# theEricMa/TriplaneTurbo

Measured on AMD Instinct MI355X. Metric: rendered rays/sec (fwd+bwd) at 256x256 rays x 128 samples, higher is better.
Workload: dtype f32 (fp32-grade: exact 3-piece fp16 operand split, 6 x v_mfma_f32_32x32x16_f16 per k-step, fp32 accumulation)

## Files before the change

### triplaneturbo_amd/csrc/tt_backward.hip

```cpp
#include "tt_backward_common.h"

struct BwdGeoParams {
    const float* packed;
    MlpPtrs w;
    const float* rays_o;
    const float* rays_d;
    const float* t_starts;
    const float* t_ends;
    tt_render_cfg cfg;
    TileGeom geom;
    long long n_items;
    int* queue;
    const float* ws;
    int n_copies;
    float* grad_packed;
    MlpGradPtrs grads;
    unsigned long long* phase_cycles;
};

#define GEO_SCRATCH_FLOATS (2 * 64 * XS)
#define GOFF_W1T LDS_GEO_FLOATS
#define GOFF_W2T (GOFF_W1T + IMG16_FLOATS(32, 64))
#define LDS_GEO16_FLOATS (GOFF_W2T + IMG16_FLOATS(64, 64))
#define GLO_W1 LDS_GEO16_FLOATS
#define GLO_W2 (GLO_W1 + LO16_FLOATS(64, 32))
#define GLO_W1T (GLO_W2 + LO16_FLOATS(64, 64))
#define GLO_W2T (GLO_W1T + LO16_FLOATS(32, 64))
#define LDS_GEO3_FLOATS (GLO_W2T + LO16_FLOATS(64, 64))
template <int PREC>
struct GeoWFloats {
    static constexpr int value = PREC == PREC_S3 ? LDS_GEO3_FLOATS : LDS_GEO16_FLOATS;
};

template <int PREC, bool WG16, bool STATS = false>
__global__ __launch_bounds__(256, 1) void k_decode_bwd_geo(BwdGeoParams p) {
    constexpr bool EXACT = PREC == PREC_F32;
    constexpr int NT = PrecNT<PREC>::value, WF = GeoWFloats<PREC>::value;
    __shared__ __attribute__((aligned(16))) float L[WF + 4 * (GEO_SCRATCH_FLOATS + SCATTER_TAG_INTS)];
    {
        MlpPtrs w = p.w;
        stage_weights<PREC, 64, 32>(L + OFF_W1, L + GLO_W1, w.w1);
        stage_weights<PREC, 64, 64>(L + OFF_W2, L + GLO_W2, w.w2);
        lds_load_matrix(L + OFF_W3, w.w3, 1, 64, 64);
        stage_weights_t<PREC, 64, 32>(L + GOFF_W1T, L + GLO_W1T, w.w1);
        stage_weights_t<PREC, 64, 64>(L + GOFF_W2T, L + GLO_W2T, w.w2);
    }
    const tt_render_cfg& cfg = p.cfg;
    float sA1 = 1.f, sU = 1.f, sA2 = 1.f, sV = 1.f;
    if (WG16) {
        const unsigned* bnd = reinterpret_cast<const unsigned*>(p.queue) + TT_SLOT_BOUNDS;
        const float Pm = __builtin_bit_cast(float, bnd[TT_BOUND_PLANES]), Sb = __builtin_bit_cast(float, bnd[TT_BOUND_UP0]),
                    Gb = __builtin_bit_cast(float, bnd[TT_BOUND_UP1]);
        unsigned* word = reinterpret_cast<unsigned*>(L + WF);
        const int t = threadIdx.x;
        float w1row = 0.f, a1col = 0.f, w3abs = 0.f;
        if (t < 64) {
            for (int c = 0; c < 32; ++c) w1row += __builtin_fabsf(p.w.w1[t * 32 + c]);
            for (int r = 0; r < 64; ++r) a1col += __builtin_fabsf(p.w.w2[r * 64 + t]) * __builtin_fabsf(p.w.w3[r]);
            w3abs = __builtin_fabsf(p.w.w3[t]);
        }
        const float W1max = block_max(w1row, word), A1max = block_max(a1col, word), A2max = block_max(w3abs, word);
        const float jsum = (0.5f * cfg.plane_w + 0.5f * cfg.plane_h) / cfg.radius;
        const float Fmax = 3.f * Pm, H1max = W1max * Fmax;
        const float Umax = Fmax * (Sb + 2.f * jsum * Gb), QBmax = Fmax * 2.f * jsum * Gb;
        const float Vmax = Sb * H1max + W1max * QBmax;
        sA1 = wg16_scale(A1max);
        sU = wg16_scale(Umax);
        sA2 = wg16_scale(A2max);
        sV = wg16_scale(Vmax);
    }
    const TileGeom& tg = p.geom;
    const int lane = threadIdx.x & 63, i = lane & 31, hi = lane >> 5, wave_in_blk = threadIdx.x >> 6;
    float* Xs = L + WF + wave_in_blk * (GEO_SCRATCH_FLOATS + SCATTER_TAG_INTS);
    float* Ys = Xs + 64 * XS;
    int* tags = reinterpret_cast<int*>(Ys + 64 * XS);
    scatter_init_tags(tags, lane);
    __syncthreads();
    const int S = cfg.n_samples;
    ItemQueue iq = item_queue(p.queue, tg.n_blocks, tg.n_chunks, tg.unit);
    const int H = cfg.plane_h, W = cfg.plane_w;
    const size_t HW = (size_t)H * W;
    const size_t plane_stride = 6 * HW * TT_C;
    const float ju = 0.5f * W / cfg.radius, jv = 0.5f * H / cfg.radius;
    float* const grad_out =
        p.grad_packed + (size_t)(blockIdx.x % (unsigned)p.n_copies) * cfg.n_prompts * plane_stride;
    const unsigned grad_bytes =
        TT_DBG(cfg.flags, TT_DBG_NO_ATOMICS) ? 0u : (unsigned)(cfg.n_prompts * plane_stride * sizeof(float));

    const TileStats st = STATS ? tile_stats(cfg.stats) : TileStats{nullptr};
    f32x16 accW1[2][1] = {{ZERO16}, {ZERO16}};
    f32x16 accW2[2][2] = {{ZERO16, ZERO16}, {ZERO16, ZERO16}};
    float accw3 = 0.f;
#ifdef TT_TUNING
    unsigned long long ph_acc[20] = {0, 0, 0, 0, 0, 0, 0, 0, 0, 0, 0, 0, 0, 0, 0, 0, 0, 0, 0, 0};
    unsigned long long ph_t = __builtin_amdgcn_s_memtime();
#endif

#pragma nounroll
    for (;;) {
        long long b;
        int ck;
        if (!item_pop(iq, tg.order, tg.n_chunks, b, ck)) break;
        if (b >= tg.n_blocks) continue;
        bool ray_ok;
        const long long ray = tile_ray(tg, b, i, ray_ok);
        const float ray_okf = tt_opaque(ray_ok ? 1.f : 0.f);
        const int ks = i % tg.sb;
        const int view = (int)(ray / cfg.rays_per_view);
        const size_t pofs = (size_t)(view / cfg.views_per_prompt) * plane_stride;
        const float ox = p.rays_o[ray * 3 + 0], oy = p.rays_o[ray * 3 + 1], oz = p.rays_o[ray * 3 + 2];
        const float dx = p.rays_d ? p.rays_d[ray * 3 + 0] : 0.f, dy = p.rays_d ? p.rays_d[ray * 3 + 1] : 0.f,
                    dz = p.rays_d ? p.rays_d[ray * 3 + 2] : 0.f;
        const int s_end = (ck + 1) * tg.chunk < S ? (ck + 1) * tg.chunk : S;
        struct StepIn {
            f32x4 up;
            float ts, te;
        };
        auto load_step = [&](int sb0) {
            StepIn r;
            const int si = sb0 + ks;
            const long long sidx = ray * S + (si < S ? si : S - 1);
            r.up = *reinterpret_cast<const f32x4*>(p.ws + sidx * 4);
            r.ts = p.rays_d ? p.t_starts[sidx] : 0.f;
            r.te = p.rays_d ? p.t_ends[sidx] : 0.f;
            return r;
        };
        StepIn in = load_step(ck * tg.chunk), in_next;
#pragma nounroll
        for (int sb0 = ck * tg.chunk; sb0 < s_end; sb0 += tg.sb, in = in_next) {
            in_next = load_step(sb0 + tg.sb);
            const int si = sb0 + ks;
            const bool rvalid = ray_ok && si < s_end;
            const float vf = ray_okf * (si < s_end ? 1.f : 0.f);
            const float sbar = in.up[0] * vf, gbx = in.up[1] * vf, gby = in.up[2] * vf, gbz = in.up[3] * vf;
            tile_stat(st, TT_STAT_VISITED);
            TT_PHASE(0);
            if (!__any(!((__builtin_fabsf(sbar) + __builtin_fabsf(gbx)) + (__builtin_fabsf(gby) + __builtin_fabsf(gbz)) <=
                         cfg.skip_eps_geo)))
                continue;
            float tm, px, py, pz;
            sample_position(ox, oy, oz, dx, dy, dz, in.ts, in.te, tm, px, py, pz);
            const float X = scale_coord(px, cfg.radius), Y = scale_coord(py, cfg.radius),
                        Z = scale_coord(pz, cfg.radius);
            float f[16], u[16];
            bool anyp[3];
            const bool any = __any(gather_geo_bwd_c(p.packed, (unsigned)(pofs / TT_C), H, W, X, Y, Z, rvalid, sbar, gbx,
                                                    gby, gbz, ju, jv, lane, Xs, f, u, anyp,
                                                    tile_stat_ptr(st, TT_STAT_INBOUNDS)));
            TT_PHASE(1);
            if (!any) continue;
            tile_stat(st, TT_STAT_EXECUTED);
            float h1[32], h2[32], a2[32], a1[32], q[16], u1, u2;
            mvx<PREC, 64, 32, true>(L + OFF_W1, L + GLO_W1, f, h1, i, hi, 1.f, &u1);
#pragma unroll
            for (int r = 0; r < 32; ++r) h1[r] = fmaxf(h1[r], 0.f);
            mvx<PREC, 64, 64, true>(L + OFF_W2, L + GLO_W2, h1, h2, i, hi, u1, &u2);
#pragma unroll
            for (int r = 0; r < 32; ++r) h2[r] = fmaxf(h2[r], 0.f);
#pragma unroll
            for (int g = 0; g < 8; ++g) {
                f32x4 w3 = *reinterpret_cast<const f32x4*>(L + OFF_W3 + 8 * g + 4 * hi);
#pragma unroll
                for (int e2 = 0; e2 < 4; ++e2) a2[4 * g + e2] = h2[4 * g + e2] > 0.f ? w3[e2] : 0.f;
            }
            Split16<64, PAIR_SEQ, NT> a2s, a1s;
            float ua1 = 1.f;
            if (WG16) {
                split16_vec<64, PAIR_SEQ, NT>(a2, sA2, a2s);
                mv16_pre<64, 64, true, NT>(L + GOFF_W2T, a2s, 1.f / sA2, a1, i, hi, &ua1, L + GLO_W2T);
            } else {
                mvtx_copy<PREC, 64, 64, 64>(L + GOFF_W2T, L + GLO_W2T, L + OFF_W2, a2, a1, i, hi);
            }
#pragma unroll
            for (int r = 0; r < 32; ++r) a1[r] = h1[r] > 0.f ? a1[r] : 0.f;
            if (WG16) {
                split16_vec<64, PAIR_SEQ, NT>(a1, sA1 * ua1, a1s);
                mv16_pre<32, 64, false, NT>(L + GOFF_W1T, a1s, 1.f / sA1, q, i, hi, nullptr, L + GLO_W1T);
            } else {
                mvtx_copy<PREC, 32, 64, 32>(L + GOFF_W1T, L + GLO_W1T, L + OFF_W1, a1, q, i, hi);
            }
            TT_PHASE(3);
            {
                float qb[16];
#pragma unroll
                for (int r = 0; r < 16; ++r) qb[r] = fmaf(-sbar, f[r], u[r]);
                const bool region = WG16 ? true : cfg.flags >= 0;
                const bool do_wgrad = region && !TT_DBG(cfg.flags, TT_DBG_NO_WGRAD);
                if (do_wgrad) {
                    if (WG16) {
                        stage_rows16_pre<64>(Xs, a1s, i, hi);
                        stage_rows16<32>(Ys, u, i, hi, sU);
                        wgrad16<64, 32>(accW1, Xs, Ys, i, hi);
                    } else {
                        stage_rows<64>(Xs, a1, i, hi);
                        stage_rows<32>(Ys, u, i, hi);
                        wgrad<64, 32>(accW1, Xs, Ys, i, hi);
                    }
                }
                TT_PHASE(7);
                float t1[32];
                mvx<PREC, 64, 32>(L + OFF_W1, L + GLO_W1, qb, t1, i, hi);
#pragma unroll
                for (int r = 0; r < 32; ++r) t1[r] = h1[r] > 0.f ? t1[r] : 0.f;
                float v[32];
#pragma unroll
                for (int r = 0; r < 32; ++r) v[r] = fmaf(sbar * u1, h1[r], t1[r]);
                TT_PHASE(4);
                if (do_wgrad) {
                    if (WG16) {
                        stage_rows16_pre<64>(Xs, a2s, i, hi);
                        stage_rows16<64>(Ys, v, i, hi, sV);
                        wgrad16<64, 64>(accW2, Xs, Ys, i, hi);
                    } else {
                        stage_rows<64>(Xs, a2, i, hi);
                        stage_rows<64>(Ys, v, i, hi);
                        wgrad<64, 64>(accW2, Xs, Ys, i, hi);
                    }
                }
                TT_PHASE(8);
                float t2[32];
                mvx<PREC, 64, 64>(L + OFF_W2, L + GLO_W2, t1, t2, i, hi);
#pragma unroll
                for (int r = 0; r < 32; ++r) t2[r] = fmaf(sbar * u2, h2[r], h2[r] > 0.f ? t2[r] : 0.f);
                stage_rows<64>(Xs, t2, i, hi);
                accw3 += rowsum32(Xs, lane);
                TT_PHASE(5);
                if (region && !TT_DBG(cfg.flags, TT_DBG_NO_SCATTER)) {
                    scatter_clear<EXACT>(Xs, lane);
                    float* Qs = Xs + SCATTER_M_FLOATS;
                    TT_PHASE(9);
                    const int tex0 = (int)(pofs / TT_C);
                    scatter_planes<EXACT>(grad_out, grad_bytes, Qs, Xs, tags, Qs + 32 * 33, i, hi,
                                          [&](int pl, PlaneRefs& refs) {
                        Corners c;
                        float coef[4];
                        geo_corner_coefs(pl, H, W, X, Y, Z, rvalid, sbar, gbx, gby, gbz, ju, jv, c, coef);
                        int aoff[4];
#pragma unroll
                        for (int q4 = 0; q4 < 4; ++q4) aoff[q4] = tex0 + (int)(pl * HW) + c.off[q4];
                        refs = plane_refs<!EXACT>(coef, aoff, c.hs, hi);
#pragma unroll
                        for (int r = 0; r < 16; ++r) Qs[i * 33 + LIDX(r, hi)] = q[r] * refs.qs;
                    }
#ifdef TT_TUNING
                    , ph_acc + 14
#endif
                    );
                    TT_PHASE(10);
                }
            }
        }
    }
#ifdef TT_TUNING
    TT_PHASE(11);
    if (p.phase_cycles && lane == 0)
        for (int k = 0; k < 20; ++k) atomicAdd(p.phase_cycles + 20 + k, ph_acc[k]);
#endif
    __syncthreads();
    int parity = 0;
    flush_wgrad_reduced<64, 32>(L, parity, accW1, p.grads.w1, wave_in_blk, lane, 1.f / sA1, 1.f / sU);
    flush_wgrad_reduced<64, 64>(L, parity, accW2, p.grads.w2, wave_in_blk, lane, 1.f / sA2, 1.f / sV);
    atomicAdd(p.grads.w3 + lane, accw3);
    tile_stats_flush(st);
}

#ifdef TT_TUNING
unsigned long long* g_phase_cycles = nullptr;
extern "C" int tt_tuning_phase_cycles(unsigned long long* out40) {
    if (!g_phase_cycles) {
        if (hipMalloc((void**)&g_phase_cycles, 40 * sizeof(unsigned long long)) != hipSuccess) return -4;
        if (hipMemset(g_phase_cycles, 0, 40 * sizeof(unsigned long long)) != hipSuccess) return -4;
    }
    if (hipDeviceSynchronize() != hipSuccess) return -4;
    if (out40 && hipMemcpy(out40, g_phase_cycles, 40 * sizeof(unsigned long long), hipMemcpyDeviceToHost) != hipSuccess)
        return -4;
    return hipMemset(g_phase_cycles, 0, 40 * sizeof(unsigned long long)) == hipSuccess ? 0 : -4;
}
#endif
static void launch_bwd_geo(const BwdGeoParams& p0, long long blocks, hipStream_t s) {
    BwdGeoParams p = p0;
#ifdef TT_TUNING
    p.phase_cycles = g_phase_cycles;
#else
    p.phase_cycles = nullptr;
#endif
    const int prec = tt_prec_of_r(p.cfg.flags);
#define LAUNCH_GEO(PREC_, WG_)                                                                                        \
    do {                                                                                                              \
        if (p.cfg.stats)                                                                                              \
            hipLaunchKernelGGL((k_decode_bwd_geo<PREC_, WG_, true>), dim3((unsigned)blocks), dim3(256), 0, s, p);     \
        else                                                                                                          \
            hipLaunchKernelGGL((k_decode_bwd_geo<PREC_, WG_>), dim3((unsigned)blocks), dim3(256), 0, s, p);           \
    } while (0)
    if (use_wg16(p.cfg)) {
        unsigned* bnd = reinterpret_cast<unsigned*>(p.queue) + TT_SLOT_BOUNDS;
        launch_planes_bound(p.packed, p.cfg, 0, bnd + TT_BOUND_PLANES, s);
        const long long n = p.cfg.n_rays * p.cfg.n_samples;
        hipLaunchKernelGGL(k_absmax4, dim3(absmax_blocks(n), 1), dim3(256), 0, s, reinterpret_cast<const f32x4*>(p.ws), n, n,
                           bnd + TT_BOUND_UP0, bnd + TT_BOUND_UP1);
        if (prec == PREC_S3)
            LAUNCH_GEO(PREC_S3, true);
        else
            LAUNCH_GEO(PREC_S2, true);
    } else {
        LAUNCH_GEO(PREC_F32, false);
    }
#undef LAUNCH_GEO
}
int tt_launch_march_bwd(const float* rays_d, const float* t_starts, const float* t_ends, const tt_render_cfg* cfg,
                        const float* sdf, const float* sdf_grad, const float* features, const float* trans,
                        const float* opacity, const float* depth, const float* g_opacity, const float* g_depth,
                        const float* g_rgb_fg, const float* g_z_variance, const float* g_normal_acc,
                        const float* g_weights, const float* g_sdf, const float* g_sdf_grad, float* g_inv_std_rays,
                        float* ws, hipStream_t stream);

extern "C" int tt_render_bwd_geo(const float* packed, const tt_mlp_weights* w, const float* rays_o,
                                 const float* rays_d, const float* t_starts, const float* t_ends,
                                 const tt_render_cfg* cfg, const float* opacity, const float* depth,
                                 const float* trans, const float* sdf, const float* sdf_grad, const float* features,
                                 const float* g_opacity, const float* g_depth, const float* g_rgb_fg,
                                 const float* g_z_variance, const float* g_normal_acc, const float* g_weights,
                                 const float* g_sdf, const float* g_sdf_grad, float* g_inv_std_rays, float* workspace,
                                 float* grad_packed, const tt_mlp_grads* grads, void* stream) {
    int st = tt_validate_cfg(cfg);
    if (st != TT_OK) return st;
    if (!packed || !w || !rays_o || !rays_d || !t_starts || !t_ends || !opacity || !depth || !trans || !sdf ||
        !sdf_grad || !features || !workspace || !grad_packed || !grads)
        return TT_ERR_BAD_ARG;
    if (!w->w1 || !w->w2 || !w->w3 || !grads->w1 || !grads->w2 || !grads->w3) return TT_ERR_BAD_ARG;
    if (grad_buffer_too_large(cfg)) return TT_ERR_UNSUPPORTED;
    int cus = tt_num_cus();
    if (cus <= 0) return TT_ERR_DEVICE;
    hipStream_t s = (hipStream_t)stream;
    st = tt_launch_march_bwd(rays_d, t_starts, t_ends, cfg, sdf, sdf_grad, features, trans, opacity, depth, g_opacity,
                             g_depth, g_rgb_fg, g_z_variance, g_normal_acc, g_weights, g_sdf, g_sdf_grad, g_inv_std_rays,
                             workspace, s);
    if (st != TT_OK) return st;
    BwdGeoParams p;
    p.packed = packed;
    p.w = to_ptrs(w);
    p.rays_o = rays_o;
    p.rays_d = rays_d;
    p.t_starts = t_starts;
    p.t_ends = t_ends;
    p.cfg = *cfg;
    p.cfg.flags |= debug_flags();
    p.ws = workspace;
    p.grad_packed = grad_packed;
    p.n_copies = cfg->grad_copies > 0 ? cfg->grad_copies : 1;
    p.grads = to_gptrs(grads);
    p.n_items = tt_make_geom(cfg, 4LL * cus, &p.geom, 1);
    long long blocks = persistent_blocks(p.n_items, cus);
    if (p.n_items > (1LL << 30)) return TT_ERR_UNSUPPORTED;
    p.queue = tt_queue_counters(s);
    if (!p.queue) return TT_ERR_DEVICE;
    launch_bwd_geo(p, blocks, s);
    return tt_check_launch();
}

__global__ void k_interleave_ws(const float* __restrict__ g_sdf, const float* __restrict__ g_sdf_grad,
                                float* __restrict__ ws, long long n) {
    const long long i = (long long)blockIdx.x * blockDim.x + threadIdx.x;
    if (i >= n) return;
    f32x4 o = {g_sdf ? g_sdf[i] : 0.f, g_sdf_grad ? g_sdf_grad[i * 3 + 0] : 0.f,
               g_sdf_grad ? g_sdf_grad[i * 3 + 1] : 0.f, g_sdf_grad ? g_sdf_grad[i * 3 + 2] : 0.f};
    *reinterpret_cast<f32x4*>(ws + i * 4) = o;
}

extern "C" int tt_points_bwd_geo(const float* packed, const tt_mlp_weights* w, const float* points, int32_t n_batch,
                                 int64_t n_points, int32_t n_prompts, int32_t views_per_prompt, int32_t plane_h,
                                 int32_t plane_w, float radius, float sdf_bias_radius, int32_t flags,
                                 const float* g_sdf, const float* g_sdf_grad, float* workspace, float* grad_packed,
                                 const tt_mlp_grads* grads, void* stream) {
    tt_render_cfg cfg;
    int st = points_cfg(&cfg, n_batch, n_points, n_prompts, views_per_prompt, plane_h, plane_w, radius,
                        sdf_bias_radius, 1, flags);
    if (st != TT_OK) return st;
    if (grad_buffer_too_large(&cfg)) return TT_ERR_UNSUPPORTED;
    if (!packed || !w || !points || !workspace || !grad_packed || !grads || (!g_sdf && !g_sdf_grad))
        return TT_ERR_BAD_ARG;
    if (!w->w1 || !w->w2 || !w->w3 || !grads->w1 || !grads->w2 || !grads->w3) return TT_ERR_BAD_ARG;
    int cus = tt_num_cus();
    if (cus <= 0) return TT_ERR_DEVICE;
    hipStream_t s = (hipStream_t)stream;
    const long long n = cfg.n_rays;
    hipLaunchKernelGGL(k_interleave_ws, dim3((unsigned)((n + 255) / 256)), dim3(256), 0, s, g_sdf, g_sdf_grad,
                       workspace, n);
    st = tt_check_launch();
    if (st != TT_OK) return st;
    BwdGeoParams p;
    p.packed = packed;
    p.w = to_ptrs(w);
    p.rays_o = points;
    p.rays_d = nullptr;
    p.t_starts = nullptr;
    p.t_ends = nullptr;
    p.cfg = cfg;
    p.ws = workspace;
    p.grad_packed = grad_packed;
    p.n_copies = 1;
    p.grads = to_gptrs(grads);
    p.n_items = tt_make_geom(&cfg, 4LL * cus, &p.geom, 1);
    if (p.n_items > (1LL << 30)) return TT_ERR_UNSUPPORTED;
    long long blocks = persistent_blocks(p.n_items, cus);
    p.queue = tt_queue_counters(s);
    if (!p.queue) return TT_ERR_DEVICE;
    launch_bwd_geo(p, blocks, s);
    return tt_check_launch();
}
```

### triplaneturbo_amd/csrc/tt_mfma16.h

```cpp
#pragma once
#include "tt_device.h"

typedef _Float16 h8_t __attribute__((ext_vector_type(8)));
typedef _Float16 h2_t __attribute__((ext_vector_type(2)));
typedef _Float16 half_t;
typedef float f2_t __attribute__((ext_vector_type(2)));

#define IMG16_FLOATS(ROWS, K) ((ROWS) * ((K) + 4))
#define LO16_FLOATS(ROWS, K) ((ROWS) * ((K) / 2 + 4))


__device__ __forceinline__ h2_t cvt_pk16(float a, float b) {
    unsigned r;
    asm("v_cvt_pk_f16_f32 %0, %1, %2" : "=v"(r) : "v"(a), "v"(b));
    return __builtin_bit_cast(h2_t, r);
}

__device__ __forceinline__ void split_pair(float a, float b, unsigned& hi, unsigned& lo) {
    asm("v_cvt_pk_f16_f32 %0, %2, %3\n\t"
        "v_fma_mix_f32 %2, %2, 1.0, -%0 op_sel_hi:[0,0,1]\n\t"
        "v_fma_mix_f32 %3, %3, 1.0, -%0 op_sel:[0,0,1] op_sel_hi:[0,0,1]\n\t"
        "v_cvt_pk_f16_f32 %1, %2, %3"
        : "=&v"(hi), "=v"(lo), "+v"(a), "+v"(b));
}
__device__ __forceinline__ void split_pair(float a, float b, h2_t& hi, h2_t& lo) {
    unsigned h, l;
    split_pair(a, b, h, l);
    hi = __builtin_bit_cast(h2_t, h);
    lo = __builtin_bit_cast(h2_t, l);
}

__device__ __forceinline__ void split_pair3(float a, float b, unsigned& hi, unsigned& mid, unsigned& lo) {
    asm("v_cvt_pk_f16_f32 %0, %3, %4\n\t"
        "v_fma_mix_f32 %3, %3, 1.0, -%0 op_sel_hi:[0,0,1]\n\t"
        "v_fma_mix_f32 %4, %4, 1.0, -%0 op_sel:[0,0,1] op_sel_hi:[0,0,1]\n\t"
        "v_cvt_pk_f16_f32 %1, %3, %4\n\t"
        "v_fma_mix_f32 %3, %3, 1.0, -%1 op_sel_hi:[0,0,1]\n\t"
        "v_fma_mix_f32 %4, %4, 1.0, -%1 op_sel:[0,0,1] op_sel_hi:[0,0,1]\n\t"
        "v_cvt_pk_f16_f32 %2, %3, %4"
        : "=&v"(hi), "=&v"(mid), "=&v"(lo), "+v"(a), "+v"(b));
}
__device__ __forceinline__ void split_pair3(float a, float b, h2_t& hi, h2_t& mid, h2_t& lo) {
    unsigned h, m, l;
    split_pair3(a, b, h, m, l);
    hi = __builtin_bit_cast(h2_t, h);
    mid = __builtin_bit_cast(h2_t, m);
    lo = __builtin_bit_cast(h2_t, l);
}

__device__ __forceinline__ void split16(float v, half_t& hi, half_t& lo) {
    const h2_t p = cvt_pk16(v, 0.f);
    hi = p.x;
    const h2_t q = cvt_pk16(v - (float)hi, 0.f);
    lo = q.x;
}
__device__ __forceinline__ void split16_3(float v, half_t& hi, half_t& mid, half_t& lo) {
    split16(v, hi, mid);
    const h2_t q = cvt_pk16((v - (float)hi) - (float)mid, 0.f);
    lo = q.x;
}

template <int ROWS, int K, bool TRANSPOSED, int NT = 2>
__device__ __forceinline__ void stage_image16(float* dst_f, const float* __restrict__ src, int ld, float* lo_f = nullptr) {
    half_t* dst = reinterpret_cast<half_t*>(dst_f);
    half_t* dlo = reinterpret_cast<half_t*>(lo_f);
    constexpr int RS = 2 * K + 8, RSL = K + 8;
    unsigned* slot = reinterpret_cast<unsigned*>(dst_f + K);
    if (threadIdx.x == 0) *slot = 0u;
    __syncthreads();
    unsigned mb = 0u;
    for (int e = threadIdx.x; e < ROWS * K; e += blockDim.x) {
        const unsigned b = __builtin_bit_cast(unsigned, src[e]) & 0x7fffffffu;
        mb = b > mb ? b : mb;
    }
    atomicMax(slot, mb);
    __syncthreads();
    int E = (int)(*slot >> 23);
    E = E < 16 ? 16 : (E > 240 ? 240 : E);
    const float sc = __builtin_bit_cast(float, (unsigned)(268 - E) << 23);
    const float un = __builtin_bit_cast(float, (unsigned)(E - 14) << 23);
    __syncthreads();
    for (int e = threadIdx.x; e < ROWS * K; e += blockDim.x) {
        const int R = e / K, c = e - R * K;
        const float v = (TRANSPOSED ? src[(size_t)c * ld + R] : src[(size_t)R * ld + c]) * sc;
        half_t hi, lo, l3 = (half_t)0.f;
        if (NT == 3)
            split16_3(v, hi, lo, l3);
        else
            split16(v, hi, lo);
        const int s = c >> 4, w = c & 15;
        const int h = (w >> 2) & 1, j = (w & 3) + 4 * (w >> 3);
        half_t* p = dst + (size_t)R * RS + (size_t)(4 * s + h) * 8 + j;
        p[0] = hi;
        p[16] = lo;
        if (NT == 3) {
            const int hf = c >= K / 2 ? 1 : 0, s2 = (c - hf * (K / 2)) >> 4;
            dlo[(size_t)R * RSL + (size_t)(4 * s2 + h) * 8 + j + 16 * hf] = l3;
        }
    }
    for (int R = threadIdx.x; R < ROWS; R += blockDim.x) dst_f[(size_t)R * (K + 4) + K] = un;
}

#ifndef TT_MV16_FENCE
#define TT_MV16_FENCE 0
#endif

template <int MT, int NT>
__device__ __forceinline__ void mfma_terms(f32x16 (&acc)[MT], const h8_t (&a0)[MT], const h8_t (&a1)[MT],
                                           const h8_t (&a2)[MT], const h8_t& b0, const h8_t& b1, const h8_t& b2) {
    if constexpr (NT == 3) {
#pragma unroll
        for (int m = 0; m < MT; ++m) acc[m] = __builtin_amdgcn_mfma_f32_32x32x16_f16(a0[m], b2, acc[m], 0, 0, 0);
#pragma unroll
        for (int m = 0; m < MT; ++m) acc[m] = __builtin_amdgcn_mfma_f32_32x32x16_f16(a2[m], b0, acc[m], 0, 0, 0);
#pragma unroll
        for (int m = 0; m < MT; ++m) acc[m] = __builtin_amdgcn_mfma_f32_32x32x16_f16(a1[m], b1, acc[m], 0, 0, 0);
#pragma unroll
        for (int m = 0; m < MT; ++m) acc[m] = __builtin_amdgcn_mfma_f32_32x32x16_f16(a0[m], b1, acc[m], 0, 0, 0);
#pragma unroll
        for (int m = 0; m < MT; ++m) acc[m] = __builtin_amdgcn_mfma_f32_32x32x16_f16(a1[m], b0, acc[m], 0, 0, 0);
#pragma unroll
        for (int m = 0; m < MT; ++m) acc[m] = __builtin_amdgcn_mfma_f32_32x32x16_f16(a0[m], b0, acc[m], 0, 0, 0);
    } else {
#pragma unroll
        for (int m = 0; m < MT; ++m) acc[m] = __builtin_amdgcn_mfma_f32_32x32x16_f16(a0[m], b0, acc[m], 0, 0, 0);
#pragma unroll
        for (int m = 0; m < MT; ++m) acc[m] = __builtin_amdgcn_mfma_f32_32x32x16_f16(a0[m], b1, acc[m], 0, 0, 0);
#pragma unroll
        for (int m = 0; m < MT; ++m) acc[m] = __builtin_amdgcn_mfma_f32_32x32x16_f16(a1[m], b0, acc[m], 0, 0, 0);
    }
}
template <int NT, bool SCALED>
__device__ __forceinline__ void split_bfrag(float x0, float x1, float sc, int d, h8_t& b0, h8_t& b1, h8_t& b2) {
    const f2_t ab = {x0, x1};
    const f2_t as = SCALED ? ab * sc : ab;
    h2_t p, q, r;
    if constexpr (NT == 3)
        split_pair3(as.x, as.y, p, q, r);
    else
        split_pair(as.x, as.y, p, q);
    b0[2 * d] = p.x;
    b0[2 * d + 1] = p.y;
    b1[2 * d] = q.x;
    b1[2 * d + 1] = q.y;
    if constexpr (NT == 3) {
        b2[2 * d] = r.x;
        b2[2 * d + 1] = r.y;
    }
}
template <int K>
__device__ __forceinline__ h8_t lo_frag(const half_t* lrow, int m, int s) {
    constexpr int RSL = K + 8, KH = K / 32;
    return *reinterpret_cast<const h8_t*>(lrow + (size_t)(32 * m) * RSL + 32 * (s % KH) + 16 * (s / KH));
}

template <int NOUT, int NIN, bool SCALED = true, bool RAW = false, int NT = 2>
__device__ __forceinline__ void mv16(const float* img_f, const float (&x)[NIN / 2], float (&y)[NOUT / 2], int i,
                                     int hi, float xf = 1.f, float* yf = nullptr, const float* lo_f = nullptr) {
    constexpr int MT = NOUT / 32, KS = NIN / 16, RS = 2 * NIN + 8;
    const half_t* row = reinterpret_cast<const half_t*>(img_f) + (size_t)i * RS + 8 * hi;
    const half_t* lrow = reinterpret_cast<const half_t*>(lo_f) + (size_t)i * (NIN + 8) + 8 * hi;
    const float wun = img_f[(size_t)i * (NIN + 4) + NIN];
    float sc = 1.f, un = wun;
    if (SCALED) {
        float m = 0.f;
#pragma unroll
        for (int r = 0; r < NIN / 2; ++r) m = fmaxf(m, __builtin_fabsf(x[r]));
        m = fmaxf(m, __shfl_xor(m, 32));
        int E = (int)(__builtin_bit_cast(unsigned, m) >> 23);
        E = E < 16 ? 16 : (E > 240 ? 240 : E);
        sc = __builtin_bit_cast(float, (unsigned)(268 - E) << 23);
        un = wun * __builtin_bit_cast(float, (unsigned)(E - 14) << 23);
    }
    un *= xf;
    f32x16 acc[MT];
#pragma unroll
    for (int m = 0; m < MT; ++m)
        acc[m] = f32x16{0.f, 0.f, 0.f, 0.f, 0.f, 0.f, 0.f, 0.f, 0.f, 0.f, 0.f, 0.f, 0.f, 0.f, 0.f, 0.f};
    if (TT_MV16_FENCE) __builtin_amdgcn_sched_barrier(0);
#pragma unroll
    for (int s = 0; s < KS; ++s) {
        h8_t bh, bl, bt;
#pragma unroll
        for (int j = 0; j < 4; ++j) split_bfrag<NT, SCALED>(x[8 * s + 2 * j], x[8 * s + 2 * j + 1], sc, j, bh, bl, bt);
        h8_t ah[MT], al[MT], at[MT];
#pragma unroll
        for (int m = 0; m < MT; ++m) {
            const half_t* a = row + (size_t)(32 * m) * RS + 32 * s;
            ah[m] = *reinterpret_cast<const h8_t*>(a);
            al[m] = *reinterpret_cast<const h8_t*>(a + 16);
            if constexpr (NT == 3) at[m] = lo_frag<NIN>(lrow, m, s);
        }
        mfma_terms<MT, NT>(acc, ah, al, at, bh, bl, bt);
    }
    if (RAW) *yf = un;
#pragma unroll
    for (int m = 0; m < MT; ++m)
#pragma unroll
        for (int k = 0; k < 16; ++k) y[16 * m + k] = RAW ? acc[m][k] : acc[m][k] * un;
}

#define PAIR_SEQ 0
#define PAIR_TR 1
template <int PAIR>
__device__ __forceinline__ constexpr int pair_reg(int t, int which) {
    return PAIR == PAIR_SEQ ? 2 * t + which : 8 * (t >> 2) + ((t & 3) >> 1) + 4 * (t & 1) + 2 * which;
}
template <int N, int PAIR = PAIR_SEQ, int NT = 2>
struct Split16 {
    unsigned h[N / 4], l[N / 4];
    unsigned t[NT == 3 ? N / 4 : 1];
};
template <int N, int PAIR, int NT>
__device__ __forceinline__ void split16_vec(const float (&x)[N / 2], float sc, Split16<N, PAIR, NT>& o) {
#pragma unroll
    for (int t = 0; t < N / 4; ++t) {
        const f2_t ab = {x[pair_reg<PAIR>(t, 0)], x[pair_reg<PAIR>(t, 1)]};
        const f2_t as = ab * sc;
        if constexpr (NT == 3)
            split_pair3(as.x, as.y, o.h[t], o.l[t], o.t[t]);
        else
            split_pair(as.x, as.y, o.h[t], o.l[t]);
    }
}
template <int NOUT, int NIN, bool RAW = false, int NT = 2>
__device__ __forceinline__ void mv16_pre(const float* img_f, const Split16<NIN, PAIR_SEQ, NT>& x, float un_x,
                                         float (&y)[NOUT / 2], int i, int hi, float* yf = nullptr,
                                         const float* lo_f = nullptr) {
    constexpr int MT = NOUT / 32, KS = NIN / 16, RS = 2 * NIN + 8;
    const half_t* row = reinterpret_cast<const half_t*>(img_f) + (size_t)i * RS + 8 * hi;
    const half_t* lrow = reinterpret_cast<const half_t*>(lo_f) + (size_t)i * (NIN + 8) + 8 * hi;
    const float un = img_f[(size_t)i * (NIN + 4) + NIN] * un_x;
    f32x16 acc[MT];
#pragma unroll
    for (int m = 0; m < MT; ++m)
        acc[m] = f32x16{0.f, 0.f, 0.f, 0.f, 0.f, 0.f, 0.f, 0.f, 0.f, 0.f, 0.f, 0.f, 0.f, 0.f, 0.f, 0.f};
    typedef unsigned u4_t __attribute__((ext_vector_type(4)));
#pragma unroll
    for (int s = 0; s < KS; ++s) {
        const h8_t bh = __builtin_bit_cast(h8_t, u4_t{x.h[4 * s], x.h[4 * s + 1], x.h[4 * s + 2], x.h[4 * s + 3]});
        const h8_t bl = __builtin_bit_cast(h8_t, u4_t{x.l[4 * s], x.l[4 * s + 1], x.l[4 * s + 2], x.l[4 * s + 3]});
        h8_t bt;
        if constexpr (NT == 3)
            bt = __builtin_bit_cast(h8_t, u4_t{x.t[4 * s], x.t[4 * s + 1], x.t[4 * s + 2], x.t[4 * s + 3]});
        h8_t ah[MT], al[MT], at[MT];
#pragma unroll
        for (int m = 0; m < MT; ++m) {
            const half_t* a = row + (size_t)(32 * m) * RS + 32 * s;
            ah[m] = *reinterpret_cast<const h8_t*>(a);
            al[m] = *reinterpret_cast<const h8_t*>(a + 16);
            if constexpr (NT == 3) at[m] = lo_frag<NIN>(lrow, m, s);
        }
        mfma_terms<MT, NT>(acc, ah, al, at, bh, bl, bt);
    }
    if (RAW) *yf = un;
#pragma unroll
    for (int m = 0; m < MT; ++m)
#pragma unroll
        for (int k = 0; k < 16; ++k) y[16 * m + k] = RAW ? acc[m][k] : acc[m][k] * un;
}

typedef short sv4_t __attribute__((__vector_size__(4 * sizeof(short))));
typedef __attribute__((address_space(3))) sv4_t lds_sv4_t;

template <int KM>
__device__ __forceinline__ const lds_sv4_t* tr_lane_base(const float* img_f, int col0, int lane) {
    constexpr int RS = 2 * KM + 8;
    const int L = lane & 15, g1 = (lane >> 4) & 1, hh = lane >> 5, j = L >> 2, q = L & 3;
    const int r1 = 2 * (j & 1) + 8 * (j >> 1) + 4 * hh;
    const int off = r1 * RS + 32 * ((col0 >> 4) + g1) + 8 * (q & 1) + 4 * (q >> 1);
    return (const lds_sv4_t*)(reinterpret_cast<const half_t*>(img_f) + off);
}
template <int KM>
__device__ __forceinline__ h8_t tr_frag(const lds_sv4_t* base, int ks, int m, int term) {
    constexpr int RS = 2 * KM + 8;
    const int off4 = (16 * ks * RS + 64 * m + 16 * term) / 4;
    const sv4_t a = __builtin_amdgcn_ds_read_tr16_b64_v4i16(const_cast<lds_sv4_t*>(base) + off4);
    const sv4_t b = __builtin_amdgcn_ds_read_tr16_b64_v4i16(const_cast<lds_sv4_t*>(base) + off4 + RS / 4);
    typedef short sv8_t __attribute__((__vector_size__(8 * sizeof(short))));
    const sv8_t ab = __builtin_shufflevector(a, b, 0, 1, 2, 3, 4, 5, 6, 7);
    return __builtin_bit_cast(h8_t, ab);
}

template <int KM>
__device__ __forceinline__ const lds_sv4_t* tr_lane_base_lo(const float* lo_f, int col0, int m, int lane) {
    constexpr int RSL = KM + 8, KH = KM / 32;
    const int L = lane & 15, g1 = (lane >> 4) & 1, hh = lane >> 5, j = L >> 2, q = L & 3;
    const int r1 = 2 * (j & 1) + 8 * (j >> 1) + 4 * hh;
    const int cb0 = (col0 >> 4) + 2 * m, cb1 = cb0 + 1;
    const int b0 = 32 * (cb0 % KH) + 16 * (cb0 / KH), b1 = 32 * (cb1 % KH) + 16 * (cb1 / KH);
    const int off = r1 * RSL + (g1 ? b1 : b0) + 8 * (q & 1) + 4 * (q >> 1);
    return (const lds_sv4_t*)(reinterpret_cast<const half_t*>(lo_f) + off);
}
template <int KM>
__device__ __forceinline__ h8_t tr_frag_lo(const lds_sv4_t* base_m, int ks) {
    constexpr int RSL = KM + 8;
    const int off4 = (16 * ks * RSL) / 4;
    const sv4_t a = __builtin_amdgcn_ds_read_tr16_b64_v4i16(const_cast<lds_sv4_t*>(base_m) + off4);
    const sv4_t b = __builtin_amdgcn_ds_read_tr16_b64_v4i16(const_cast<lds_sv4_t*>(base_m) + off4 + RSL / 4);
    typedef short sv8_t __attribute__((__vector_size__(8 * sizeof(short))));
    const sv8_t ab = __builtin_shufflevector(a, b, 0, 1, 2, 3, 4, 5, 6, 7);
    return __builtin_bit_cast(h8_t, ab);
}

template <int NOUT, int NIN, int KM, bool SCALED = true, bool RAW = false, int NT = 2>
__device__ __forceinline__ void mv16t(const float* img_f, int col0, const float (&x)[NIN / 2], float (&y)[NOUT / 2],
                                      int lane, float xf = 1.f, float* yf = nullptr, const float* lo_f = nullptr) {
    constexpr int MT = NOUT / 32, KS = NIN / 16;
    const lds_sv4_t* base = tr_lane_base<KM>(img_f, col0, lane);
    const lds_sv4_t* base_lo[MT];
    if constexpr (NT == 3) {
#pragma unroll
        for (int m = 0; m < MT; ++m) base_lo[m] = tr_lane_base_lo<KM>(lo_f, col0, m, lane);
    }
    const float wun = img_f[KM];
    float sc = 1.f, un = wun;
    if (SCALED) {
        float m = 0.f;
#pragma unroll
        for (int r = 0; r < NIN / 2; ++r) m = fmaxf(m, __builtin_fabsf(x[r]));
        m = fmaxf(m, __shfl_xor(m, 32));
        int E = (int)(__builtin_bit_cast(unsigned, m) >> 23);
        E = E < 16 ? 16 : (E > 240 ? 240 : E);
        sc = __builtin_bit_cast(float, (unsigned)(268 - E) << 23);
        un = wun * __builtin_bit_cast(float, (unsigned)(E - 14) << 23);
    }
    un *= xf;
    f32x16 acc[MT];
#pragma unroll
    for (int m = 0; m < MT; ++m)
        acc[m] = f32x16{0.f, 0.f, 0.f, 0.f, 0.f, 0.f, 0.f, 0.f, 0.f, 0.f, 0.f, 0.f, 0.f, 0.f, 0.f, 0.f};
    if (TT_MV16_FENCE) __builtin_amdgcn_sched_barrier(0);
#pragma unroll
    for (int s = 0; s < KS; ++s) {
        h8_t bh, bl, bt;
#pragma unroll
        for (int d = 0; d < 4; ++d)
            split_bfrag<NT, SCALED>(x[8 * s + pair_reg<PAIR_TR>(d, 0)], x[8 * s + pair_reg<PAIR_TR>(d, 1)], sc, d, bh, bl, bt);
        h8_t ah[MT], al[MT], at[MT];
#pragma unroll
        for (int m = 0; m < MT; ++m) {
            ah[m] = tr_frag<KM>(base, s, m, 0);
            al[m] = tr_frag<KM>(base, s, m, 1);
            if constexpr (NT == 3) at[m] = tr_frag_lo<KM>(base_lo[m], s);
        }
        mfma_terms<MT, NT>(acc, ah, al, at, bh, bl, bt);
    }
    if (RAW) *yf = un;
#pragma unroll
    for (int m = 0; m < MT; ++m)
#pragma unroll
        for (int k = 0; k < 16; ++k) y[16 * m + k] = RAW ? acc[m][k] : acc[m][k] * un;
}

enum { PREC_S2 = 0, PREC_F32 = 1, PREC_S3 = 2 };
template <int PREC>
struct PrecNT {
    static constexpr int value = PREC == PREC_S3 ? 3 : 2;
};
template <int PREC, int ROWS, int K>
__device__ __forceinline__ void stage_weights(float* dst_f, float* lo_f, const float* __restrict__ src) {
    if constexpr (PREC == PREC_F32) {
        lds_load_matrix(dst_f, src, ROWS, K, K + 4);
    } else {
        stage_image16<ROWS, K, false, PrecNT<PREC>::value>(dst_f, src, K, lo_f);
    }
}

template <int PREC, int ROWS_SRC, int K_SRC>
__device__ __forceinline__ void stage_weights_t(float* dst_f, float* lo_f, const float* __restrict__ src) {
    if constexpr (PREC != PREC_F32) stage_image16<K_SRC, ROWS_SRC, true, PrecNT<PREC>::value>(dst_f, src, K_SRC, lo_f);
}

template <int PREC, int NOUT, int NIN, bool RAW = false>
__device__ __forceinline__ void mvx(const float* img, const float* lo, const float (&x)[NIN / 2], float (&y)[NOUT / 2],
                                    int i, int hi, float xf = 1.f, float* yf = nullptr) {
    if constexpr (PREC == PREC_F32) {
        mv_fwd<NOUT, NIN>(img, x, y, i, hi);
        if (RAW) *yf = 1.f;
    } else {
        mv16<NOUT, NIN, true, RAW, PrecNT<PREC>::value>(img, x, y, i, hi, xf, yf, lo);
    }
}
template <int PREC, int NOUT, int NIN, int KM, bool RAW = false>
__device__ __forceinline__ void mvtx_copy(const float* img_t, const float* lo_t, const float* img,
                                          const float (&x)[NIN / 2], float (&y)[NOUT / 2], int i, int hi, float xf = 1.f,
                                          float* yf = nullptr) {
    if constexpr (PREC == PREC_F32) {
        mv_bwd<NOUT, NIN, KM + 4>(img, x, y, i, hi);
        if (RAW) *yf = 1.f;
    } else {
        mv16<NOUT, NIN, true, RAW, PrecNT<PREC>::value>(img_t, x, y, i, hi, xf, yf, lo_t);
    }
}
template <int PREC, int NOUT, int NIN, int KM, bool RAW = false>
__device__ __forceinline__ void mvtx(const float* img, const float* lo, int col0, const float (&x)[NIN / 2],
                                     float (&y)[NOUT / 2], int i, int hi, float xf = 1.f, float* yf = nullptr) {
    if constexpr (PREC == PREC_F32) {
        mv_bwd<NOUT, NIN, KM + 4>(img + col0, x, y, i, hi);
        if (RAW) *yf = 1.f;
    } else {
        mv16t<NOUT, NIN, KM, true, RAW, PrecNT<PREC>::value>(img, col0, x, y, 32 * hi + i, xf, yf, lo);
    }
}

#define LO_W1 LDS_W_FLOATS
#define LO_W2 (LO_W1 + LO16_FLOATS(64, 32))
#define LO_V1 (LO_W2 + LO16_FLOATS(64, 64))
#define LO_V2 (LO_V1 + LO16_FLOATS(64, 96))
#define LDS_W3P_FLOATS (LO_V2 + LO16_FLOATS(64, 64))
template <int PREC>
struct FwdWFloats {
    static constexpr int value = PREC == PREC_S3 ? LDS_W3P_FLOATS : LDS_W_FLOATS;
};
#define TT_PREC_OF(exact, split2) ((exact) ? PREC_F32 : ((split2) ? PREC_S2 : PREC_S3))
```

Before: 7.277 million.

## Pair forward and tangent matvecs to share weight fragment loads

Fuses the W1 and W2 forward matvecs with the later qb/t1 matvecs through the same weights into one paired MFMA routine. Each A fragment loaded from LDS feeds both accumulators, and the B-operand split for the next k-step is issued ahead of the current MFMAs. This removes duplicate LDS weight reads and raises MFMA density. In exchange it raises register pressure from two accumulator sets and longer-lived t1/t2/v arrays, which could reduce occupancy or cause spills.

```diff
diff --git a/triplaneturbo_amd/csrc/tt_backward.hip b/triplaneturbo_amd/csrc/tt_backward.hip
--- a/triplaneturbo_amd/csrc/tt_backward.hip
+++ b/triplaneturbo_amd/csrc/tt_backward.hip
@@ -1,3 +1,6 @@
+#ifndef TT_MV16_FENCE
+#define TT_MV16_FENCE 1
+#endif
 #include "tt_backward_common.h"
 
 struct BwdGeoParams {
@@ -150,13 +153,27 @@
             TT_PHASE(1);
             if (!any) continue;
             tile_stat(st, TT_STAT_EXECUTED);
-            float h1[32], h2[32], a2[32], a1[32], q[16], u1, u2;
-            mvx<PREC, 64, 32, true>(L + OFF_W1, L + GLO_W1, f, h1, i, hi, 1.f, &u1);
-#pragma unroll
-            for (int r = 0; r < 32; ++r) h1[r] = fmaxf(h1[r], 0.f);
-            mvx<PREC, 64, 64, true>(L + OFF_W2, L + GLO_W2, h1, h2, i, hi, u1, &u2);
-#pragma unroll
-            for (int r = 0; r < 32; ++r) h2[r] = fmaxf(h2[r], 0.f);
+            float h1[32], h2[32], a2[32], a1[32], q[16], v[32], u1, u2;
+            {
+                float qb[16], t1[32], t2[32];
+#pragma unroll
+                for (int r = 0; r < 16; ++r) qb[r] = fmaf(-sbar, f[r], u[r]);
+                mvx_pair<PREC, 64, 32, true, false>(L + OFF_W1, L + GLO_W1, f, h1, 1.f, &u1, qb, t1, 1.f, nullptr, i, hi);
+#pragma unroll
+                for (int r = 0; r < 32; ++r) h1[r] = fmaxf(h1[r], 0.f);
+#pragma unroll
+                for (int r = 0; r < 32; ++r) t1[r] = h1[r] > 0.f ? t1[r] : 0.f;
+                mvx_pair<PREC, 64, 64, true, false>(L + OFF_W2, L + GLO_W2, h1, h2, u1, &u2, t1, t2, 1.f, nullptr, i, hi);
+#pragma unroll
+                for (int r = 0; r < 32; ++r) h2[r] = fmaxf(h2[r], 0.f);
+#pragma unroll
+                for (int r = 0; r < 32; ++r) v[r] = fmaf(sbar * u1, h1[r], t1[r]);
+#pragma unroll
+                for (int r = 0; r < 32; ++r) t2[r] = fmaf(sbar * u2, h2[r], h2[r] > 0.f ? t2[r] : 0.f);
+                stage_rows<64>(Xs, t2, i, hi);
+                accw3 += rowsum32(Xs, lane);
+            }
+            TT_PHASE(3);
 #pragma unroll
             for (int g = 0; g < 8; ++g) {
                 f32x4 w3 = *reinterpret_cast<const f32x4*>(L + OFF_W3 + 8 * g + 4 * hi);
@@ -179,11 +196,8 @@
             } else {
                 mvtx_copy<PREC, 32, 64, 32>(L + GOFF_W1T, L + GLO_W1T, L + OFF_W1, a1, q, i, hi);
             }
-            TT_PHASE(3);
+            TT_PHASE(4);
             {
-                float qb[16];
-#pragma unroll
-                for (int r = 0; r < 16; ++r) qb[r] = fmaf(-sbar, f[r], u[r]);
                 const bool region = WG16 ? true : cfg.flags >= 0;
                 const bool do_wgrad = region && !TT_DBG(cfg.flags, TT_DBG_NO_WGRAD);
                 if (do_wgrad) {
@@ -198,14 +212,6 @@
                     }
                 }
                 TT_PHASE(7);
-                float t1[32];
-                mvx<PREC, 64, 32>(L + OFF_W1, L + GLO_W1, qb, t1, i, hi);
-#pragma unroll
-                for (int r = 0; r < 32; ++r) t1[r] = h1[r] > 0.f ? t1[r] : 0.f;
-                float v[32];
-#pragma unroll
-                for (int r = 0; r < 32; ++r) v[r] = fmaf(sbar * u1, h1[r], t1[r]);
-                TT_PHASE(4);
                 if (do_wgrad) {
                     if (WG16) {
                         stage_rows16_pre<64>(Xs, a2s, i, hi);
@@ -218,13 +224,6 @@
                     }
                 }
                 TT_PHASE(8);
-                float t2[32];
-                mvx<PREC, 64, 64>(L + OFF_W2, L + GLO_W2, t1, t2, i, hi);
-#pragma unroll
-                for (int r = 0; r < 32; ++r) t2[r] = fmaf(sbar * u2, h2[r], h2[r] > 0.f ? t2[r] : 0.f);
-                stage_rows<64>(Xs, t2, i, hi);
-                accw3 += rowsum32(Xs, lane);
-                TT_PHASE(5);
                 if (region && !TT_DBG(cfg.flags, TT_DBG_NO_SCATTER)) {
                     scatter_clear<EXACT>(Xs, lane);
                     float* Qs = Xs + SCATTER_M_FLOATS;
diff --git a/triplaneturbo_amd/csrc/tt_mfma16.h b/triplaneturbo_amd/csrc/tt_mfma16.h
--- a/triplaneturbo_amd/csrc/tt_mfma16.h
+++ b/triplaneturbo_amd/csrc/tt_mfma16.h
@@ -154,6 +154,18 @@
     return *reinterpret_cast<const h8_t*>(lrow + (size_t)(32 * m) * RSL + 32 * (s % KH) + 16 * (s / KH));
 }
 
+template <int NIN>
+__device__ __forceinline__ void sample_scale(const float (&x)[NIN / 2], float wun, float& sc, float& un) {
+    float m = 0.f;
+#pragma unroll
+    for (int r = 0; r < NIN / 2; ++r) m = fmaxf(m, __builtin_fabsf(x[r]));
+    m = fmaxf(m, __shfl_xor(m, 32));
+    int E = (int)(__builtin_bit_cast(unsigned, m) >> 23);
+    E = E < 16 ? 16 : (E > 240 ? 240 : E);
+    sc = __builtin_bit_cast(float, (unsigned)(268 - E) << 23);
+    un = wun * __builtin_bit_cast(float, (unsigned)(E - 14) << 23);
+}
+
 template <int NOUT, int NIN, bool SCALED = true, bool RAW = false, int NT = 2>
 __device__ __forceinline__ void mv16(const float* img_f, const float (&x)[NIN / 2], float (&y)[NOUT / 2], int i,
                                      int hi, float xf = 1.f, float* yf = nullptr, const float* lo_f = nullptr) {
@@ -162,16 +174,7 @@
     const half_t* lrow = reinterpret_cast<const half_t*>(lo_f) + (size_t)i * (NIN + 8) + 8 * hi;
     const float wun = img_f[(size_t)i * (NIN + 4) + NIN];
     float sc = 1.f, un = wun;
-    if (SCALED) {
-        float m = 0.f;
-#pragma unroll
-        for (int r = 0; r < NIN / 2; ++r) m = fmaxf(m, __builtin_fabsf(x[r]));
-        m = fmaxf(m, __shfl_xor(m, 32));
-        int E = (int)(__builtin_bit_cast(unsigned, m) >> 23);
-        E = E < 16 ? 16 : (E > 240 ? 240 : E);
-        sc = __builtin_bit_cast(float, (unsigned)(268 - E) << 23);
-        un = wun * __builtin_bit_cast(float, (unsigned)(E - 14) << 23);
-    }
+    if (SCALED) sample_scale<NIN>(x, wun, sc, un);
     un *= xf;
     f32x16 acc[MT];
 #pragma unroll
@@ -198,6 +201,72 @@
     for (int m = 0; m < MT; ++m)
 #pragma unroll
         for (int k = 0; k < 16; ++k) y[16 * m + k] = RAW ? acc[m][k] : acc[m][k] * un;
+}
+
+template <int MT, int NT>
+__device__ __forceinline__ void mfma_terms_pair(f32x16 (&acca)[MT], f32x16 (&accb)[MT], const h8_t (&a0)[MT],
+                                                const h8_t (&a1)[MT], const h8_t (&a2)[MT], const h8_t (&ba)[3],
+                                                const h8_t (&bb)[3]) {
+    constexpr int TA3[6] = {0, 2, 1, 0, 1, 0}, TB3[6] = {2, 0, 1, 1, 0, 0}, TA2[3] = {0, 0, 1}, TB2[3] = {0, 1, 0};
+#pragma unroll
+    for (int t = 0; t < (NT == 3 ? 6 : 3); ++t) {
+        const int pa = NT == 3 ? TA3[t] : TA2[t], pb = NT == 3 ? TB3[t] : TB2[t];
+        const h8_t(&a)[MT] = pa == 0 ? a0 : (pa == 1 ? a1 : a2);
+#pragma unroll
+        for (int m = 0; m < MT; ++m) acca[m] = __builtin_amdgcn_mfma_f32_32x32x16_f16(a[m], ba[pb], acca[m], 0, 0, 0);
+#pragma unroll
+        for (int m = 0; m < MT; ++m) accb[m] = __builtin_amdgcn_mfma_f32_32x32x16_f16(a[m], bb[pb], accb[m], 0, 0, 0);
+    }
+}
+template <int NOUT, int NIN, bool RAWA, bool RAWB, int NT>
+__device__ __forceinline__ void mv16_pair(const float* img_f, const float* lo_f, const float (&xa)[NIN / 2],
+                                          float (&ya)[NOUT / 2], float xfa, float* yfa, const float (&xb)[NIN / 2],
+                                          float (&yb)[NOUT / 2], float xfb, float* yfb, int i, int hi) {
+    constexpr int MT = NOUT / 32, KS = NIN / 16, RS = 2 * NIN + 8;
+    const half_t* row = reinterpret_cast<const half_t*>(img_f) + (size_t)i * RS + 8 * hi;
+    const half_t* lrow = reinterpret_cast<const half_t*>(lo_f) + (size_t)i * (NIN + 8) + 8 * hi;
+    const float wun = img_f[(size_t)i * (NIN + 4) + NIN];
+    float sca, una, scb, unb;
+    sample_scale<NIN>(xa, wun, sca, una);
+    sample_scale<NIN>(xb, wun, scb, unb);
+    una *= xfa;
+    unb *= xfb;
+    f32x16 acca[MT], accb[MT];
+#pragma unroll
+    for (int m = 0; m < MT; ++m) acca[m] = accb[m] = f32x16{0.f, 0.f, 0.f, 0.f, 0.f, 0.f, 0.f, 0.f, 0.f, 0.f, 0.f, 0.f, 0.f, 0.f, 0.f, 0.f};
+    if (TT_MV16_FENCE) __builtin_amdgcn_sched_barrier(0);
+    h8_t ba[2][3], bb[2][3];
+    auto split_step = [&](int s, h8_t(&fa)[3], h8_t(&fb)[3]) {
+#pragma unroll
+        for (int j = 0; j < 4; ++j) {
+            split_bfrag<NT, true>(xa[8 * s + 2 * j], xa[8 * s + 2 * j + 1], sca, j, fa[0], fa[1], fa[2]);
+            split_bfrag<NT, true>(xb[8 * s + 2 * j], xb[8 * s + 2 * j + 1], scb, j, fb[0], fb[1], fb[2]);
+        }
+    };
+    split_step(0, ba[0], bb[0]);
+#pragma unroll
+    for (int s = 0; s < KS; ++s) {
+        h8_t ah[MT], al[MT], at[MT];
+#pragma unroll
+        for (int m = 0; m < MT; ++m) {
+            const half_t* a = row + (size_t)(32 * m) * RS + 32 * s;
+            ah[m] = *reinterpret_cast<const h8_t*>(a);
+            al[m] = *reinterpret_cast<const h8_t*>(a + 16);
+            if constexpr (NT == 3) at[m] = lo_frag<NIN>(lrow, m, s);
+        }
+        if (s + 1 < KS) split_step(s + 1, ba[(s + 1) & 1], bb[(s + 1) & 1]);
+        mfma_terms_pair<MT, NT>(acca, accb, ah, al, at, ba[s & 1], bb[s & 1]);
+    }
+    if (TT_MV16_FENCE) __builtin_amdgcn_sched_barrier(0);
+    if (RAWA) *yfa = una;
+    if (RAWB) *yfb = unb;
+#pragma unroll
+    for (int m = 0; m < MT; ++m)
+#pragma unroll
+        for (int k = 0; k < 16; ++k) {
+            ya[16 * m + k] = RAWA ? acca[m][k] : acca[m][k] * una;
+            yb[16 * m + k] = RAWB ? accb[m][k] : accb[m][k] * unb;
+        }
 }
 
 #define PAIR_SEQ 0
@@ -315,16 +384,7 @@
     }
     const float wun = img_f[KM];
     float sc = 1.f, un = wun;
-    if (SCALED) {
-        float m = 0.f;
-#pragma unroll
-        for (int r = 0; r < NIN / 2; ++r) m = fmaxf(m, __builtin_fabsf(x[r]));
-        m = fmaxf(m, __shfl_xor(m, 32));
-        int E = (int)(__builtin_bit_cast(unsigned, m) >> 23);
-        E = E < 16 ? 16 : (E > 240 ? 240 : E);
-        sc = __builtin_bit_cast(float, (unsigned)(268 - E) << 23);
-        un = wun * __builtin_bit_cast(float, (unsigned)(E - 14) << 23);
-    }
+    if (SCALED) sample_scale<NIN>(x, wun, sc, un);
     un *= xf;
     f32x16 acc[MT];
 #pragma unroll
@@ -380,6 +440,17 @@
         if (RAW) *yf = 1.f;
     } else {
         mv16<NOUT, NIN, true, RAW, PrecNT<PREC>::value>(img, x, y, i, hi, xf, yf, lo);
+    }
+}
+template <int PREC, int NOUT, int NIN, bool RAWA = false, bool RAWB = false>
+__device__ __forceinline__ void mvx_pair(const float* img, const float* lo, const float (&xa)[NIN / 2],
+                                         float (&ya)[NOUT / 2], float xfa, float* yfa, const float (&xb)[NIN / 2],
+                                         float (&yb)[NOUT / 2], float xfb, float* yfb, int i, int hi) {
+    if constexpr (PREC == PREC_F32) {
+        mvx<PREC, NOUT, NIN, RAWA>(img, lo, xa, ya, i, hi, xfa, yfa);
+        mvx<PREC, NOUT, NIN, RAWB>(img, lo, xb, yb, i, hi, xfb, yfb);
+    } else {
+        mv16_pair<NOUT, NIN, RAWA, RAWB, PrecNT<PREC>::value>(img, lo, xa, ya, xfa, yfa, xb, yb, xfb, yfb, i, hi);
     }
 }
 template <int PREC, int NOUT, int NIN, int KM, bool RAW = false>
```

Result: slower. 7.200 million (-1.1%).
